# Chenxu1103/UNET-

Measured on AMD Instinct MI355X. Metric: frames/sec 512x512 3-class UNet++ inference; mask vs CPU reference, higher is better.
Workload: dtype f16 (MFMA operands split hi+lo, 3 MFMAs per product, f32 accumulate); 1 GPU; UNet++ 3-class 512x512 batch=16/GPU fp16-MFMA on 1 MI355X, synthetic frames, f32 NCHW in HBM -> uint8 mask in HBM; arch=nested, precision=exact, frames_per_gpu=16, global_batch=16, micro_batch=16, parallelism=frame-sharded x1, weights replicated (RCCL bcast)

## Files before the change

unet-_amd/csrc/tapmm_ws.h:

```cpp
#pragma once
#include "conv3x3_ws.h"

namespace unetpp {

struct TapmmArgs {
  const half_t* low;
  const half_t* wpk;
  float* y;
  int N, hw, K, Nv;
#ifdef UNETPP_WS_DBG
  int dbg;
#endif
};

struct TapmmCfg {
  static constexpr int NT = 512, NCONS = 4, NPROD = 4;
  static constexpr int TM = 256, TN = 128, MT = 4, NTL = 2;
  static constexpr int A_BYTES = TM * 64, B_BYTES = TN * 64, STAGE_BYTES = A_BYTES + B_BYTES;
  static constexpr int SLOTS = 6, LDS_BYTES = SLOTS * STAGE_BYTES;
  static constexpr int A_PIECES = A_BYTES / 1024, B_PIECES = B_BYTES / 1024;
  static constexpr int A_IT = A_PIECES / NPROD, B_IT = B_PIECES / NPROD, DMA_PER_STAGE = A_IT + B_IT;
  static constexpr int AHEAD = 4;
  static_assert(LDS_BYTES <= 160 * 1024 && AHEAD + 2 <= SLOTS, "ring");
};

template <bool X8>
__global__ __launch_bounds__(512, 2) void tapmm_ws_kernel(TapmmArgs a) {
  using C = TapmmCfg;
  extern __shared__ __attribute__((aligned(16))) char smem[];
  touch_kernarg_lines<TapmmArgs>();
  const int tid = threadIdx.x, lane = tid & 63;
  const int wave = __builtin_amdgcn_readfirstlane(tid >> 6);
  const unsigned lds_base = (unsigned)(unsigned long)(lds_char_t*)smem;
  const int mtiles_img = (a.hw + C::TM - 1) / C::TM;
  const int ntiles = a.Nv / C::TN;
  const int total_tiles = a.N * mtiles_img * ntiles;
  const int nst = a.K / 16;
  const int G = (int)gridDim.x;
  const int slot = (G % 8 == 0) ? ((int)blockIdx.x % 8) * (G / 8) + (int)blockIdx.x / 8 : (int)blockIdx.x;
  auto decode = [&](int t, int& n, int& q0, int& vt) {
    vt = t % ntiles; t /= ntiles;
    const int mt = t % mtiles_img;
    n = t / mtiles_img;
    q0 = mt * C::TM;
  };
  if (slot >= total_tiles) return;
  if (wave >= C::NCONS) {
    const int pw = wave - C::NCONS;
    constexpr unsigned OOB = 0x80000000u;
    const unsigned blk_bytes = (unsigned)a.hw * 64u;
    int it_tile = slot, it_s = 0;
    int in_, iq0, ivt;
    decode(it_tile, in_, iq0, ivt);
    auto issue = [&](int ring) {
#ifdef UNETPP_WS_DBG
      if (a.dbg & TAPMM_NO_DMA) {
        if (++it_s == nst) { it_s = 0; it_tile += G; if (it_tile < total_tiles) decode(it_tile, in_, iq0, ivt); }
        return;
      }
#endif
      const __amdgpu_buffer_rsrc_t rs = __builtin_amdgcn_make_buffer_rsrc(
          (void*)(a.low + (size_t)in_ * (a.K / 16) * a.hw * 32), 0, (int)((a.K / 16) * blk_bytes), 0x00020000);
      const unsigned dstA = lds_base + ring * C::STAGE_BYTES;
#pragma unroll
      for (int it = 0; it < C::A_IT; ++it) {
        const int piece = pw + it * C::NPROD;
        const int q = iq0 + piece * 16 + (lane & 15);
        const unsigned voff = q < a.hw ? (unsigned)q * 64u + (unsigned)(lane >> 4) * 16u : OOB;
        blds16(rs, voff, it_s * (int)blk_bytes, dstA + piece * 1024);
      }
      const char* wsrc = (const char*)a.wpk + ((size_t)ivt * nst + it_s) * C::B_BYTES;
#pragma unroll
      for (int it = 0; it < C::B_IT; ++it) {
        const int piece = pw + it * C::NPROD;
        glds16(wsrc + piece * 1024, lane * 16, dstA + C::A_BYTES + piece * 1024);
      }
      if (++it_s == nst) {
        it_s = 0; it_tile += G;
        if (it_tile < total_tiles) decode(it_tile, in_, iq0, ivt);
      }
    };
    int issued = 0, g = 0;
    for (int k = 0; k <= C::AHEAD && it_tile < total_tiles; ++k, ++issued) issue(issued % C::SLOTS);
    for (int tile = slot; tile < total_tiles; tile += G)
      for (int s = 0; s < nst; ++s, ++g) {
        const int later = issued - (g + 2);
        if (later >= 3) asm volatile("s_waitcnt vmcnt(18)" ::: "memory");
        else if (later == 2) asm volatile("s_waitcnt vmcnt(12)" ::: "memory");
        else if (later == 1) asm volatile("s_waitcnt vmcnt(6)" ::: "memory");
        else asm volatile("s_waitcnt vmcnt(0)" ::: "memory");
        lds_barrier();
        if (it_tile < total_tiles) { issue(issued % C::SLOTS); ++issued; }
      }
    return;
  }

  const int cw = wave, pxh = cw & 1, vh = cw >> 1;
  static_assert(C::DMA_PER_STAGE == 6, "vmcnt ladder above");
  int a_off[C::MT];
#pragma unroll
  for (int mt = 0; mt < C::MT; ++mt) {
    const int px = pxh * 128 + mt * 32 + (lane & 31);
    a_off[mt] = (px >> 4) * 1024 + ((lane >> 5) * 16 + (px & 15)) * 16;
  }
  const int b_off = C::A_BYTES + (vh * 2) * 2048 + (lane >> 5) * 512 + (lane & 31) * 16;
  struct Frag { half8 ah[C::MT], al[C::MT], bh[C::NTL], bl[C::NTL]; };
  auto load_frags = [&](Frag& f, int ring) {
    const char* st = smem + ring * C::STAGE_BYTES;
#pragma unroll
    for (int mt = 0; mt < C::MT; ++mt) { f.ah[mt] = *(const half8*)(st + a_off[mt]); f.al[mt] = *(const half8*)(st + a_off[mt] + 512); }
#pragma unroll
    for (int nt = 0; nt < C::NTL; ++nt) { f.bh[nt] = *(const half8*)(st + b_off + nt * 2048); f.bl[nt] = *(const half8*)(st + b_off + nt * 2048 + 1024); }
  };
  float16v acc[C::MT][C::NTL];
  auto run_mfma = [&](const Frag& f) {
    if (WS_OFF(a.dbg, TAPMM_NO_MFMA)) return;
#pragma unroll
    for (int mt = 0; mt < C::MT; ++mt)
#pragma unroll
      for (int nt = 0; nt < C::NTL; ++nt) {
        acc[mt][nt] = __builtin_amdgcn_mfma_f32_32x32x16_f16(f.bh[nt], f.al[mt], acc[mt][nt], 0, 0, 0);
        acc[mt][nt] = __builtin_amdgcn_mfma_f32_32x32x16_f16(f.bl[nt], f.ah[mt], acc[mt][nt], 0, 0, 0);
        acc[mt][nt] = __builtin_amdgcn_mfma_f32_32x32x16_f16(f.bh[nt], f.ah[mt], acc[mt][nt], 0, 0, 0);
      }
  };

  int g = 0;
  Frag f0, f1;
  bool have_f0 = false;
  struct HFrag { half8 a[C::MT], b[C::NTL]; };
  HFrag h0, h1;
  int8v xa[C::MT], xb[C::NTL];
  auto load_h = [&](HFrag& f, int ring) {
    const char* st = smem + ring * C::STAGE_BYTES;
#pragma unroll
    for (int mt = 0; mt < C::MT; ++mt) f.a[mt] = *(const half8*)(st + a_off[mt]);
#pragma unroll
    for (int nt = 0; nt < C::NTL; ++nt) f.b[nt] = *(const half8*)(st + b_off + nt * 2048);
  };
  auto load_x = [&](int ring0, int ring1) {
    const char* s0 = smem + ring0 * C::STAGE_BYTES;
    const char* s1 = smem + ring1 * C::STAGE_BYTES;
#pragma unroll
    for (int mt = 0; mt < C::MT; ++mt) {
      const int4v lo = *(const int4v*)(s0 + a_off[mt] + 512), hi = *(const int4v*)(s1 + a_off[mt] + 512);
      xa[mt] = __builtin_shufflevector(lo, hi, 0, 1, 2, 3, 4, 5, 6, 7);
    }
#pragma unroll
    for (int nt = 0; nt < C::NTL; ++nt) {
      const int4v lo = *(const int4v*)(s0 + b_off + nt * 2048 + 1024), hi = *(const int4v*)(s1 + b_off + nt * 2048 + 1024);
      xb[nt] = __builtin_shufflevector(lo, hi, 0, 1, 2, 3, 4, 5, 6, 7);
    }
  };
  auto main_mfma = [&](const HFrag& f) {
#pragma unroll
    for (int mt = 0; mt < C::MT; ++mt)
#pragma unroll
      for (int nt = 0; nt < C::NTL; ++nt) acc[mt][nt] = __builtin_amdgcn_mfma_f32_32x32x16_f16(f.b[nt], f.a[mt], acc[mt][nt], 0, 0, 0);
  };
  auto cross_mfma = [&]() {
#pragma unroll
    for (int mt = 0; mt < C::MT; ++mt)
#pragma unroll
      for (int nt = 0; nt < C::NTL; ++nt) {
        acc[mt][nt] = __builtin_amdgcn_mfma_scale_f32_32x32x64_f8f6f4(xb[nt], xa[mt], acc[mt][nt], 0 , 1 , 0, X8_SCALE_W, 0, X8_SCALE_A);
      }
  };
  for (int tile = slot; tile < total_tiles; tile += G) {
    int n, q0, vt;
    decode(tile, n, q0, vt);
#pragma unroll
    for (int mt = 0; mt < C::MT; ++mt)
#pragma unroll
      for (int nt = 0; nt < C::NTL; ++nt)
#pragma unroll
        for (int r = 0; r < 16; ++r) acc[mt][nt][r] = 0.f;
    const bool last_tile = tile + G >= total_tiles;
    if constexpr (X8) {
      for (int s = 0; s < nst; s += 2) {
        lds_barrier();
        if (!have_f0) { load_h(h0, g % C::SLOTS); have_f0 = true; }
        load_x(g % C::SLOTS, (g + 1) % C::SLOTS);
        load_h(h1, (g + 1) % C::SLOTS);
        __builtin_amdgcn_sched_barrier(0);
        main_mfma(h0);
        __builtin_amdgcn_sched_barrier(0);
        ++g;
        lds_barrier();
        const bool more = !(last_tile && s + 2 >= nst);
        if (more) load_h(h0, (g + 1) % C::SLOTS);
        have_f0 = more;
        __builtin_amdgcn_sched_barrier(0);
        cross_mfma();
        main_mfma(h1);
        __builtin_amdgcn_sched_barrier(0);
        ++g;
      }
    } else
    for (int s = 0; s < nst; s += 2) {
      lds_barrier();
      if (!have_f0) { load_frags(f0, g % C::SLOTS); have_f0 = true; }
      load_frags(f1, (g + 1) % C::SLOTS);
      __builtin_amdgcn_sched_barrier(0);
      run_mfma(f0);
      __builtin_amdgcn_sched_barrier(0);
      ++g;
      lds_barrier();
      const bool more = !(last_tile && s + 2 >= nst);
      if (more) load_frags(f0, (g + 1) % C::SLOTS);
      have_f0 = more;
      __builtin_amdgcn_sched_barrier(0);
      run_mfma(f1);
      __builtin_amdgcn_sched_barrier(0);
      ++g;
    }
    if (WS_OFF(a.dbg, TAPMM_NO_STORE)) { if (acc[0][0][0] == 12345.f) a.y[0] = 1.f; continue; }
    const int h = lane >> 5;
#pragma unroll
    for (int mt = 0; mt < C::MT; ++mt) {
      const int q = q0 + pxh * 128 + mt * 32 + (lane & 31);
#pragma unroll
      for (int nt = 0; nt < C::NTL; ++nt) {
        const int vb = vt * (C::TN / 32) + vh * 2 + nt;
        float* dst = a.y + (((size_t)n * (a.Nv / 32) + vb) * a.hw + q) * 32 + 4 * h;
        if (q < a.hw) {
#pragma unroll
          for (int qq = 0; qq < 4; ++qq) {
            *(f32x4*)(dst + 8 * qq) = (f32x4){acc[mt][nt][4 * qq], acc[mt][nt][4 * qq + 1], acc[mt][nt][4 * qq + 2], acc[mt][nt][4 * qq + 3]};
          }
        }
      }
    }
  }
}

__global__ void tapw_pack_kernel(const float* __restrict__ w, const float* __restrict__ mult, int Cout, int Cs, int Cup,
                                 half_t* __restrict__ out, long long units, int x8) {
  const long long u = (long long)blockIdx.x * blockDim.x + threadIdx.x;
  if (u >= units) return;
  long long t = u;
  const int vv = t % 32; t /= 32;
  const int kg = t % 2; t /= 2;
  const int pl = t % 2; t /= 2;
  const int vt = t % 4; t /= 4;
  const int nst = Cup / 16;
  const int ks = t % nst; t /= nst;
  const int v128 = (int)t;
  const int v = v128 * 128 + vt * 32 + vv;
  const int tap = v / Cout, co = v - tap * Cout;
  half8 r;
  float val[8];
#pragma unroll
  for (int e = 0; e < 8; ++e) {
    const int c = ks * 16 + kg * 8 + e;
    val[e] = w[((size_t)co * (Cs + Cup) + Cs + c) * 9 + tap] * mult[co];
    const half_t hi = (half_t)val[e];
    r[e] = pl == 0 ? hi : (half_t)(val[e] - (float)hi);
  }
  if (x8 && pl == 1) {
    unsigned wd[4];
#pragma unroll
    for (int q = 0; q < 2; ++q) {
      int a8 = 0, b8 = 0;
      float hi4[4], lo4[4];
#pragma unroll
      for (int i = 0; i < 4; ++i) { hi4[i] = val[4 * q + i] * 0.015625f; lo4[i] = (val[4 * q + i] - (float)(half_t)val[4 * q + i]) * 32.0f; }
      a8 = __builtin_amdgcn_cvt_pk_fp8_f32(hi4[0], hi4[1], a8, false); a8 = __builtin_amdgcn_cvt_pk_fp8_f32(hi4[2], hi4[3], a8, true);
      b8 = __builtin_amdgcn_cvt_pk_fp8_f32(lo4[0], lo4[1], b8, false); b8 = __builtin_amdgcn_cvt_pk_fp8_f32(lo4[2], lo4[3], b8, true);
      wd[2 * q] = (unsigned)a8; wd[2 * q + 1] = (unsigned)b8;
    }
    *(u32x4*)(out + u * 8) = (u32x4){wd[0], wd[1], wd[2], wd[3]};
    return;
  }
  *(half8*)(out + u * 8) = r;
}

struct UpsumArgs {
  const float* y;
  float* z;
  int N, H, W, Cout;
};

template <int TH_>
struct UpsumCfgT {
  static constexpr int TH = TH_, TW = 32, RH = TH / 2 + 3, RW = TW / 2 + 3, RECS = RH * RW;
  static constexpr int PIECES = (RECS * 128 + 1023) / 1024, BUF_BYTES = PIECES * 1024;
  static constexpr int YTAB_BYTES = (TH + 2) * 16, LDS_BYTES = BUF_BYTES + YTAB_BYTES;
  static constexpr int ITERS = (PIECES + 3) / 4;
};
typedef UpsumCfgT<16> UpsumCfg;

template <int TB, int TH_ = 16>
__global__ __launch_bounds__(256, TB == 1 ? 4 : 1) void upsum_kernel(UpsumArgs a) {
  using C = UpsumCfgT<TH_>;
  extern __shared__ __attribute__((aligned(16))) char smem[];
  const int H = a.H, W = a.W, h = H >> 1, w = W >> 1;
  const int tid = threadIdx.x, lane = tid & 63;
  const int wave = __builtin_amdgcn_readfirstlane(tid >> 6);
  const unsigned lds_base = (unsigned)(unsigned long)(lds_char_t*)smem;
  const int tiles_x = (W + C::TW - 1) / C::TW, tiles_y = (H + C::TH - 1) / C::TH;
  int t = blockIdx.x;
  const int tx = t % tiles_x; t /= tiles_x;
  const int ty = t % tiles_y; t /= tiles_y;
  const int cb = t % (a.Cout / 32);
  const int n = t / (a.Cout / 32);
  const int y0 = ty * C::TH, x0 = tx * C::TW;
  const float sh = h > 1 ? (float)(h - 1) / (float)(H - 1) : 0.f;
  const float sw = w > 1 ? (float)(w - 1) / (float)(W - 1) : 0.f;
  const int ybase = (int)(sh * (float)max(y0 - 1, 0)), xbase = (int)(sw * (float)max(x0 - 1, 0));
  const int vblocks = 9 * a.Cout / 32;
  const size_t plane = (size_t)h * w * 128;
  unsigned voff[C::ITERS];
#pragma unroll
  for (int it = 0; it < C::ITERS; ++it) {
    const int rec = (wave + it * 4) * 8 + (lane >> 3);
    const int ry = rec / C::RW, rx = rec - ry * C::RW;
    const int yy = min(ybase + ry, h - 1), xx = min(xbase + rx, w - 1);
    voff[it] = (wave + it * 4 < C::PIECES) ? (unsigned)((yy * w + xx) * 128 + (lane & 7) * 16) : 0x80000000u;
  }
  auto stage = [&](int tap, int buf) {
    const int vb = (tap * a.Cout) / 32 + cb;
    const __amdgpu_buffer_rsrc_t rs = __builtin_amdgcn_make_buffer_rsrc((void*)((const char*)a.y + ((size_t)n * vblocks + vb) * plane), 0,
                                                                       (int)plane, 0x00020000);
#pragma unroll
    for (int it = 0; it < C::ITERS; ++it) {
      const int piece = wave + it * 4;
      if (piece < C::PIECES) blds16(rs, voff[it], 0, lds_base + buf * C::BUF_BYTES + piece * 1024);
    }
  };
  const int cq = tid & 7, col = tid >> 3;
  int xo0[3], xo1[3]; float xl0[3], xl1[3];
#pragma unroll
  for (int dx = 0; dx < 3; ++dx) {
    const int xx = x0 + col + dx - 1;
    const bool in = xx >= 0 && xx < W && x0 + col < W;
    const float fx = sw * (float)max(xx, 0);
    const int c0 = min((int)fx, w - 1), c1 = c0 + (c0 < w - 1 ? 1 : 0);
    const float l1 = fminf(fmaxf(fx - (float)c0, 0.f), 1.f);
    xo0[dx] = min(max(c0 - xbase, 0), C::RW - 1) * 128 + cq * 16;
    xo1[dx] = min(max(c1 - xbase, 0), C::RW - 1) * 128 + cq * 16;
    xl0[dx] = in ? 1.f - l1 : 0.f; xl1[dx] = in ? l1 : 0.f;
  }
  struct YRow { int o0, o1; float l0, l1; };
  YRow* ytab = (YRow*)(smem + TB * C::BUF_BYTES);
  if (tid < C::TH + 2) {
    const int yy = y0 + tid - 1;
    const bool in = yy >= 0 && yy < H;
    const float fy = sh * (float)max(yy, 0);
    const int r0 = min((int)fy, h - 1), r1 = r0 + (r0 < h - 1 ? 1 : 0);
    const float l1 = fminf(fmaxf(fy - (float)r0, 0.f), 1.f);
    YRow e;
    e.o0 = min(max(r0 - ybase, 0), C::RH - 1) * (C::RW * 128);
    e.o1 = min(max(r1 - ybase, 0), C::RH - 1) * (C::RW * 128);
    e.l0 = in ? 1.f - l1 : 0.f; e.l1 = in ? l1 : 0.f;
    ytab[tid] = e;
  }
  f32x4 sum[C::TH];
#pragma unroll
  for (int r = 0; r < C::TH; ++r) sum[r] = (f32x4){0.f, 0.f, 0.f, 0.f};

  for (int tap0 = 0; tap0 < 9; tap0 += TB) {
    __syncthreads();
#pragma unroll
    for (int t = 0; t < TB; ++t) stage(tap0 + t, t);
    asm volatile("s_waitcnt vmcnt(0)" ::: "memory");
    __syncthreads();
#pragma unroll
    for (int t = 0; t < TB; ++t) {
    const int tap = tap0 + t;
    const char* reg = smem + t * C::BUF_BYTES;
    const int dy = tap / 3, dx = tap - dy * 3;
#pragma unroll
    for (int r = 0; r < C::TH; ++r) {
      const YRow yr = ytab[r + dy];
      const f32x4 c00 = *(const f32x4*)(reg + yr.o0 + xo0[dx]), c01 = *(const f32x4*)(reg + yr.o0 + xo1[dx]);
      const f32x4 c10 = *(const f32x4*)(reg + yr.o1 + xo0[dx]), c11 = *(const f32x4*)(reg + yr.o1 + xo1[dx]);
#pragma unroll
      for (int e = 0; e < 4; ++e) {
        const float t0 = fmaf(xl1[dx], c01[e], xl0[dx] * c00[e]), t1 = fmaf(xl1[dx], c11[e], xl0[dx] * c10[e]);
        sum[r][e] += fmaf(yr.l1, t1, yr.l0 * t0);
      }
    }
    }
  }
  const int x = x0 + col;
  if (x < W) {
#pragma unroll
    for (int r = 0; r < C::TH; ++r)
      if (y0 + r < H)
        *(f32x4*)(a.z + (((size_t)n * (a.Cout / 32) + cb) * ((size_t)H * W) + (size_t)(y0 + r) * W + x) * 32 + cq * 4) = sum[r];
  }
}

}
```

unet-_amd/csrc/unetpp_abi.hip:

```cpp
#include <hip/hip_runtime.h>

#include <algorithm>
#include <cerrno>
#include <cmath>
#include <cstdarg>
#include <cstdio>
#include <cstdlib>
#include <cstring>
#include <string>
#include <map>
#include <memory>
#include <mutex>
#include <set>
#include <tuple>
#include <utility>
#include <vector>

#include "abi_common.h"
#include "aux_kernels.h"
#include "conv3x3_mfma.h"
#include "conv3x3_ws.h"
#include "convt2x2_mfma.h"
#include "tapmm_ws.h"
#include "ws_dbg_host.h"
// ... 559 lines not shown
    snprintf(nm, sizeof nm, "dec%d", l + 1);
    int da = b.tensor(std::string(nm) + "a", SB[l], l);
    int d = b.tensor(nm, SB[l], l);
    int c1 = b.conv(std::string(nm) + ".0", 2 * SB[l], u, enc[l], da);
    e->convs[c1].w_off = dec_w[l][0]; e->convs[c1].b_off = dec_b[l][0];
    int c2 = b.conv(std::string(nm) + ".2", SB[l], da, -1, d);
    e->convs[c2].w_off = dec_w[l][1]; e->convs[c2].b_off = dec_b[l][1];
    prev = d;
  }
  b.off = off;
  b.head(prev, SB[0]);
}

struct Prec {
  int P; bool x8;
  template <class K> K pick(K fast, K exact, K exact8) const { return x8 ? exact8 : P == 2 ? exact : fast; }
  const char* args() const { return pick("1", "2", "2, true"); }
  const char* head_args() const { return pick("1", "2", "3"); }
};

struct InSlice { const char* raw; int format; double bytes_per_px; };
InSlice in_slice(const void* dev_input, int in_format, int b0, size_t hw) {
  const int bpp = in_format == UNETPP_IN_F32_NCHW ? 12 : 3;
  return {(const char*)dev_input + (size_t)b0 * hw * bpp, in_format, (double)bpp};
}

struct OutSlice {
  const unetpp_outputs* o = nullptr;
  float* logits = nullptr; float* probs = nullptr;
  uint8_t* mask = nullptr; uint8_t* cable = nullptr; uint8_t* tape = nullptr;
  double bytes_per_px = 0;
};
OutSlice out_slice(const unetpp_outputs* o, int b0, int C, size_t hw) {
  OutSlice r;
  if (!o) return r;
  r.o = o;
  if (o->dev_logits) r.logits = o->dev_logits + (size_t)b0 * C * hw;
  if (o->dev_probs) r.probs = o->dev_probs + (size_t)b0 * C * hw;
  if (o->dev_mask) r.mask = o->dev_mask + (size_t)b0 * hw;
  if (o->dev_cable) r.cable = o->dev_cable + (size_t)b0 * hw;
  if (o->dev_tape) r.tape = o->dev_tape + (size_t)b0 * hw;
  r.bytes_per_px = (r.logits ? 4.0 * C : 0) + (r.probs ? 4.0 * C : 0) + (r.mask ? 1 : 0) + (r.cable ? 1 : 0) + (r.tape ? 1 : 0);
  return r;
}

struct Pass {
  unetpp_engine* e;
  hipStream_t s;
  Launcher& lx;
  int nb, b0, h, w;
  int slot;
  size_t slot_off;
  InSlice in;
  OutSlice out[4];
  bool head_done = false;
#ifdef UNETPP_WS_DBG
  WsDbgPass dbg;
#endif
  half_t* tp(int id) const { return (half_t*)(e->arena + slot_off + e->tensors[id].off); }
};

bool x8_pair9(const unetpp_engine* e, const ConvLayer& L) { return e->x8 && L.nchunks % 2 == 0; }

void run_convert(Pass& c) {
  unetpp_engine* e = c.e;
  const Prec prec{e->P, e->x8};
  const size_t total = (size_t)c.nb * c.h * c.w;
  const double bytes = (double)total * c.in.bytes_per_px + (double)total * e->P * 16;
  c.lx.run(std::string("convert_input|convert_input_kernel<") + prec.args() + ">", 0, bytes, [&] {
    hipLaunchKernelGGL(prec.pick(convert_input_kernel<1>, convert_input_kernel<2>, convert_input_kernel<2, true>), dim3((unsigned)((total + 255) / 256)),
                       dim3(256), 0, c.s, (const void*)c.in.raw, c.in.format, c.nb, c.h, c.w, c.tp(e->t_in8), e->d_status);
    return hipSuccess;
  });
}

void run_conv(Pass& c, const Op& op) {
  unetpp_engine* e = c.e;
  const ConvLayer& L = e->convs[op.idx];
  const int P = e->P, C = e->cfg.num_classes;
  const bool head = op.fuse_head && !e->keep_all && L.cout == 32;
  const OutSlice& o = c.out[0];
  ConvArgs a{};
  const int H = c.h >> L.lvl, W = c.w >> L.lvl;
  const Tensor& t0 = e->tensors[L.in];
  const int c1 = L.in2 >= 0 ? e->tensors[L.in2].C : 0;
  a.in0 = c.tp(L.in); a.in1 = L.in2 >= 0 ? c.tp(L.in2) : nullptr; a.C0 = t0.C; a.C1 = c1;
  a.wpk = e->at<half_t>(L.wpk_at); a.scale = e->at<float>(L.scale_at); a.bias = e->blob + L.b_off; a.out = c.tp(L.out);
  a.pool_out = L.do_pool ? c.tp(L.pool) : nullptr;
  a.N = c.nb; a.H = H; a.W = W; a.Cout = L.cout;
  a.status = e->d_status;
  a.zinit = L.zt >= 0 ? (const float*)c.tp(L.zt) : nullptr;
  if (e->t_kpart >= 0) { a.kpart = (float*)c.tp(e->t_kpart); a.kcnt = (unsigned*)c.tp(e->t_kcnt); }
  a.ksplit = 1;
  a.pair9 = x8_pair9(e, L) ? 1 : 0;
  if (L.c0f) {
    const ConvLayer& L1 = e->convs[e->c0f_conv1];
    a.raw_in = c.in.raw;
    a.raw_fmt = c.in.format == UNETPP_IN_F32_NCHW ? 0 : 1;
    a.c1w = e->c1w; a.c1_scale = e->at<float>(L1.scale_at); a.c1_bias = e->blob + L1.b_off;
  }
  const int mw = small_grid_rows(L, e->num_cus, c.nb, H, W, head);
  const int TH = L.WAVES * mw;
  a.tiles_x = (W + 31) / 32; a.tiles_y = (H + TH - 1) / TH;
  a.nct = L.cout / (32 * L.NW); a.nchunks = L.nchunks;
  double px = (double)c.nb * H * W;
  double flops = 2.0 * px * L.cout * (L.zt >= 0 ? t0.C : L.cin_real) * 9;
  double bytes = px * P * 2.0 * (t0.C + (L.upf ? c1 / 4.0 : c1) + (head ? 0 : L.cout)) + (L.do_pool ? px / 4 * P * 2.0 * L.cout : 0.0) + (double)L.cout * L.cin_real * 9 * 2.0 * P;
  if (L.zt >= 0) bytes += px * L.cout * 4.0 - (double)L.cout * (L.cin_real - t0.C) * 9 * 2.0 * P;
  if (L.c0f) {
    flops += 2.0 * px * 32 * 3 * 9;
    bytes += px * c.in.bytes_per_px - px * P * 2.0 * t0.C;
  }
  if (head) {
    a.head_w = e->blob + e->head_w_off; a.head_b = e->blob + e->head_b_off; a.head_C = C;
    a.logits = o.logits; a.mask = o.mask; a.cable = o.cable; a.tape = o.tape;
    a.probs = o.probs; a.rule = o.o->rule;
    a.t_cable = o.o->t_cable; a.t_tape = o.o->t_tape; a.bg_margin = o.o->bg_margin; a.ct_margin = o.o->ct_margin;
    flops += 2.0 * px * 32 * C;
    bytes += px * o.bytes_per_px;
    c.head_done = true;
  }
  const WsVariant v = ws_variant(P, e->x8, L, head, e->keep_all);
  std::string lbl;
  if (L.ws) {
    lbl = ws_label(P, e->x8, L, v);
  } else {
    char buf[160];
    auto tf = [](bool b) { return b ? "true" : "false"; };
    snprintf(buf, sizeof buf, "%s%s%s|conv3x3_bias_relu_kernel<%d, %d, %d, %d, %d, %s, %s, %s>", L.name.c_str(), L.upf ? "+up" : "", head ? "+final+argmax" : "",
             P, L.KC, L.NW, mw, L.WAVES, tf(L.do_pool), tf(head), tf(L.upf));
    lbl = buf;
  }
#ifdef UNETPP_WS_DBG
  ws_dbg_before_launch(c.dbg, a, L.name, c.s);
#endif
  c.lx.run(lbl, flops, bytes, [&] {
    return L.ws ? launch_ws(LaunchCtx{e->cfg.device, e->num_cus, e->ksplit_max, e->ksplit_min_chunks, e->ksplit_gate, c.lx.plan}, e->x8, v, a, c.s)
                : launch_conv(LaunchCtx{e->cfg.device, e->num_cus, 1, 4, 4, c.lx.plan}, P, L, mw, a, head, c.s);
  });
#ifdef UNETPP_WS_DBG
  ws_dbg_after_launch(c.dbg, a, L.name, L.ws, c.s);
#endif
}

void run_tapmm(Pass& c, const Op& op) {
  unetpp_engine* e = c.e;
  const ConvLayer& L = e->convs[op.idx];
  const int P = e->P, H = c.h >> L.lvl, W = c.w >> L.lvl;
  const int cup = L.cin_real - e->tensors[L.in].C;
  TapmmArgs t{};
  t.low = c.tp(L.low_t); t.wpk = e->at<half_t>(L.tapw_at); t.y = (float*)c.tp(L.y_t);
  t.N = c.nb; t.hw = (H >> 1) * (W >> 1); t.K = cup; t.Nv = 9 * L.cout;
#ifdef UNETPP_WS_DBG
  { const char* d = getenv("UNETPP_TAPMM_DBG"); t.dbg = d ? atoi(d) : 0; }
#endif
  const int tiles = c.nb * ((t.hw + TapmmCfg::TM - 1) / TapmmCfg::TM) * (t.Nv / TapmmCfg::TN);
  const double M = (double)c.nb * t.hw;
  char lbl[96];
  snprintf(lbl, sizeof lbl, "%s.up-gemm|tapmm_ws_kernel<%s>", L.name.c_str(), e->x8 ? "true" : "false");
  c.lx.run(lbl, 2.0 * M * cup * t.Nv, M * cup * 2.0 * P + M * t.Nv * 4.0 + (double)t.Nv * cup * 2.0 * P, [&] {
    auto k = e->x8 ? tapmm_ws_kernel<true> : tapmm_ws_kernel<false>;
    hipError_t st = allow_full_lds((const void*)k, e->cfg.device);
    if (st != hipSuccess) return st;
    const int grid = std::min(tiles, e->num_cus);
    if (c.lx.plan) { c.lx.plan[0] = grid; c.lx.plan[1] = tiles; c.lx.plan[2] = 1; c.lx.plan[3] = 0; }
    hipLaunchKernelGGL(k, dim3((unsigned)grid), dim3(TapmmCfg::NT), TapmmCfg::LDS_BYTES, c.s, t);
    return hipSuccess;
  });
}

void run_upsum(Pass& c, const Op& op) {
  unetpp_engine* e = c.e;
  const ConvLayer& L = e->convs[op.idx];
  const int H = c.h >> L.lvl, W = c.w >> L.lvl;
  UpsumArgs u{};
  u.y = (const float*)c.tp(L.y_t); u.z = (float*)c.tp(L.zt); u.N = c.nb; u.H = H; u.W = W; u.Cout = L.cout;
  unsigned blocks = (unsigned)(((W + UpsumCfg::TW - 1) / UpsumCfg::TW) * ((H + UpsumCfg::TH - 1) / UpsumCfg::TH) * (L.cout / 32) * c.nb);
  const double px = (double)c.nb * H * W;
  char lbl[96];
  const bool small = blocks <= (unsigned)e->num_cus;
  if (small) blocks = (unsigned)(((W + 31) / 32) * ((H + 3) / 4) * (L.cout / 32) * c.nb);
  snprintf(lbl, sizeof lbl, "%s.up-sum|upsum_kernel<1, %d>", L.name.c_str(), small ? 4 : 16);
  c.lx.run(lbl, px * L.cout * 9 * 8.0, px / 4 * 9 * L.cout * 4.0 + px * L.cout * 4.0, [&] {
    if (small) hipLaunchKernelGGL((upsum_kernel<1, 4>), dim3(blocks), dim3(256), UpsumCfgT<4>::LDS_BYTES, c.s, u);
    else hipLaunchKernelGGL((upsum_kernel<1, 16>), dim3(blocks), dim3(256), UpsumCfg::LDS_BYTES, c.s, u);
    return hipSuccess;
  });
}

void run_up(Pass& c, const Op& op) {
  unetpp_engine* e = c.e;
  const Tensor& low = e->tensors[op.idx];
  const Tensor& dst = e->tensors[op.out];
  const int P = e->P, H = c.h >> dst.lvl, W = c.w >> dst.lvl;
  double px = (double)c.nb * H * W;
  double bytes = px * P * 2.0 * low.C + px / 4 * P * 2.0 * low.C;
  const int nseg = (W + UP_SEG - 1) / UP_SEG;
  const int seg_w = std::min(W, UP_SEG);
  const size_t up_lds = (size_t)3 * (seg_w / 2 + 2) * P * 32;
  const int up_threads = seg_w * 2 * P >= 1024 ? 512 : (seg_w * 2 * P >= 256 ? 256 : 128);
  char nm[64];
  snprintf(nm, sizeof nm, "up%d|upsample2x_kernel<1>", dst.lvl);
  c.lx.run(nm, px * low.C * 8, bytes, [&] {
    if (P != 1) return hipErrorInvalidValue;
    hipLaunchKernelGGL(upsample2x_kernel<1>, dim3((unsigned)((H / 2) * nseg), (unsigned)(c.nb * (low.C / 16))), dim3(up_threads), up_lds, c.s, c.tp(op.idx), H, W, c.tp(op.out));
    return hipSuccess;
  });
}

void run_convt(Pass& c, const Op& op) {
  unetpp_engine* e = c.e;
  const ConvTLayer& T = e->convts[op.idx];
  const Prec prec{e->P, e->x8};
  const int P = e->P, H = c.h >> T.lvl, W = c.w >> T.lvl;
  ConvTArgs a{};
  a.in = c.tp(T.in); a.wpk = e->at<half_t>(T.wpk_at); a.scale = e->at<float>(T.scale_at); a.bias = e->blob + T.b_off; a.out = c.tp(T.out);
  a.N = c.nb; a.H = H; a.W = W; a.Cin = T.cin; a.Cout = T.cout;
  a.status = e->d_status;
  double px = (double)c.nb * H * W;
  double flops = 2.0 * px * T.cin * T.cout * 4;
  double bytes = px * P * 2.0 * (T.cin + 4.0 * T.cout) + 4.0 * T.cin * T.cout * 2.0 * P;
  dim3 grid((unsigned)(((H * W + 511) / 512) * (4 * T.cout / 64) * c.nb));
  c.lx.run(T.name + "|convt2x2_kernel<" + prec.args() + ">", flops, bytes, [&] {
    hipLaunchKernelGGL(prec.pick(convt2x2_kernel<1>, convt2x2_kernel<2>, convt2x2_kernel<2, true>), grid, dim3(256), 0, c.s, a);
    return hipSuccess;
  });
}

void run_ds(Pass& c, const Op& op) {
  unetpp_engine* e = c.e;
  const Prec prec{e->P, e->x8};
  const int k = op.idx, C = e->cfg.num_classes, P = e->P, h = c.h, w = c.w;
  const OutSlice& o = c.out[k];
  if (!o.o) return;
  const int cx = e->tensors[op.out].C, hk = h >> k, wk = w >> k;
  const double lowpx = (double)c.nb * hk * wk, px = (double)c.nb * h * w;
  const float* dsw = e->ds_w + e->ds_w_off[k];
  const char* nm = k == 3 ? "ds3_1" : k == 2 ? "ds2_2" : "ds1_3";
  float* low = e->ds_scratch[c.slot] + e->ds_scr_off[k];
  const dim3 hgrid((unsigned)((hk * wk + 255) / 256), (unsigned)c.nb);
  const size_t lds = (size_t)(C * cx + C) * sizeof(float);
  c.lx.run(std::string(nm) + "|head_generic_kernel<" + prec.head_args() + ">", 2.0 * lowpx * cx * C, lowpx * (P * 2.0 * cx + 4.0 * C), [&] {
    uint8_t* none = nullptr;
    hipLaunchKernelGGL(prec.pick(head_generic_kernel<1>, head_generic_kernel<2>, head_generic_kernel<3>), hgrid, dim3(256), lds, c.s, c.tp(op.out), cx, dsw,
                       dsw + (size_t)C * cx, C, hk, wk, low, (float*)nullptr, none, none, none, 0, 0.f, 0.f, 0.f, 0.f);
    return hipSuccess;
  });
  const float sy = (float)(hk - 1) / (float)(h - 1), sx = (float)(wk - 1) / (float)(w - 1);
  const size_t items = (size_t)c.nb * h * (w / 4);
  c.lx.run(std::string(nm) + "+up|ds_upsample_kernel", px * C * 9.0, lowpx * 4.0 * C + px * o.bytes_per_px, [&] {
    hipLaunchKernelGGL(ds_upsample_kernel, dim3((unsigned)((items + 255) / 256)), dim3(256), 0, c.s, (const float*)low, C, hk, wk, c.nb, h, w, sy, sx,
                       o.logits, o.probs, o.mask, o.cable, o.tape, o.o->rule, o.o->t_cable, o.o->t_tape, o.o->bg_margin, o.o->ct_margin);
    return hipSuccess;
  });
}

void run_head(Pass& c, const Op& op) {
  if (c.head_done) return;
  unetpp_engine* e = c.e;
  const Prec prec{e->P, e->x8};
  const OutSlice& o = c.out[0];
  const int cx = e->head_cx, C = e->cfg.num_classes;
  const size_t hw = (size_t)c.h * c.w, total = c.nb * hw;
  const dim3 grid((unsigned)((hw + 255) / 256), (unsigned)c.nb);
  const size_t lds = (size_t)(C * cx + C) * sizeof(float);
  c.lx.run(std::string("final+argmax|head_generic_kernel<") + prec.head_args() + ">", 2.0 * total * cx * C, (double)total * (e->P * 2.0 * cx + o.bytes_per_px), [&] {
    hipLaunchKernelGGL(prec.pick(head_generic_kernel<1>, head_generic_kernel<2>, head_generic_kernel<3>), grid, dim3(256), lds, c.s, c.tp(op.out), cx,
                       e->blob + e->head_w_off, e->blob + e->head_b_off, C, c.h, c.w, o.logits, o.probs, o.mask, o.cable, o.tape, o.o->rule, o.o->t_cable,
                       o.o->t_tape, o.o->bg_margin, o.o->ct_margin);
    return hipSuccess;
  });
}

}

extern "C" {

#ifndef UNETPP_SRC_HASH
#define UNETPP_SRC_HASH "unknown"
#endif
#ifdef UNETPP_WS_DBG
#define UNETPP_BUILD_TAG " +wsdbg"
#else
#define UNETPP_BUILD_TAG ""
#endif
const char* unetpp_version(void) { return "unetpp-hip 0.3.0 (gfx950) src:" UNETPP_SRC_HASH UNETPP_BUILD_TAG; }

const char* unetpp_last_error(const unetpp_engine* e) { return e ? e->err.c_str() : g_create_error.c_str(); }

size_t unetpp_weights_blob_bytes(int num_classes, int in_channels) {
  return 32 + 4 * blob_payload_floats(UNETPP_ARCH_NESTED, num_classes, in_channels);
}

size_t unetpp_weights_blob_bytes_arch(int arch, int num_classes, int in_channels) {
  if (arch != UNETPP_ARCH_NESTED && arch != UNETPP_ARCH_SIMPLE) return 0;
  return 32 + 4 * blob_payload_floats(arch, num_classes, in_channels);
}

int unetpp_create(const unetpp_config* cfg, unetpp_engine** out) {
  if (!cfg || !out) return fail(nullptr, UNETPP_E_INVALID, "null argument");
  *out = nullptr;
  if (cfg->arch != UNETPP_ARCH_NESTED && cfg->arch != UNETPP_ARCH_SIMPLE) return fail(nullptr, UNETPP_E_INVALID, "arch=%d unknown", cfg->arch);
  if (cfg->in_channels != 3) return fail(nullptr, UNETPP_E_UNSUPPORTED, "input_channels=%d unsupported (only 3)", cfg->in_channels);
  if (cfg->num_classes < 1 || cfg->num_classes > HEAD_FUSED_MAX_CLASSES)
    return fail(nullptr, UNETPP_E_INVALID, "num_classes=%d out of range [1,%d]", cfg->num_classes, HEAD_FUSED_MAX_CLASSES);
  const int mult = cfg->arch == UNETPP_ARCH_NESTED ? 16 : 8;
  if (cfg->max_batch < 1 || cfg->max_h < mult || cfg->max_w < mult || cfg->max_h % mult || cfg->max_w % mult)
// ... 445 lines not shown
```

Before: 4276 frames/s.

## Block tapmm tiles for L2 weight reuse and overlap epilogue stores with MFMAs

When the grid size is a multiple of 8, tapmm tiles are remapped so that each XCD-group of blocks walks a limited band of weight column tiles sized to about 2.5MB, aiming to keep weights resident in L2. Accumulator zeroing is folded into the first MFMA by passing a zero accumulator. Output stores become bounds-checked buffer stores interleaved with the last k-step's MFMAs, so the write-out overlaps compute. A second kernel's tile order is also remapped to group tiles per XCD with y as the fast axis. The changes add index arithmetic and scheduling complexity, and the store interleave depends on sched_barrier placement.

```diff
diff --git a/unet-_amd/csrc/tapmm_ws.h b/unet-_amd/csrc/tapmm_ws.h
--- a/unet-_amd/csrc/tapmm_ws.h
+++ b/unet-_amd/csrc/tapmm_ws.h
@@ -22,6 +22,7 @@
   static constexpr int A_IT = A_PIECES / NPROD, B_IT = B_PIECES / NPROD, DMA_PER_STAGE = A_IT + B_IT;
   static constexpr int AHEAD = 4;
   static_assert(LDS_BYTES <= 160 * 1024 && AHEAD + 2 <= SLOTS, "ring");
+  static constexpr long long W_L2 = 5 << 19;
 };
 
 template <bool X8>
@@ -38,8 +39,19 @@
   const int nst = a.K / 16;
   const int G = (int)gridDim.x;
   const int slot = (G % 8 == 0) ? ((int)blockIdx.x % 8) * (G / 8) + (int)blockIdx.x / 8 : (int)blockIdx.x;
+  const int nblk = (int)(((long long)ntiles * a.K * (C::TN * 4) + C::W_L2 - 1) / C::W_L2);
+  const int vblk = (ntiles + nblk - 1) / nblk;
+  const bool blocked = G % 8 == 0 && vblk < ntiles;
   auto decode = [&](int t, int& n, int& q0, int& vt) {
-    vt = t % ntiles; t /= ntiles;
+    if (blocked) {
+      const int g8 = G / 8, s = t % G, x = s / g8, rounds = total_tiles / G, rem = total_tiles - rounds * G;
+      const int p = x * rounds * g8 + min(rem, x * g8) + (t / G) * g8 + (s - x * g8);
+      const int span = vblk * a.N * mtiles_img, vb = p / span, r = p - vb * span;
+      const int wd = min(vblk, ntiles - vb * vblk);
+      vt = vb * vblk + r % wd; t = r / wd;
+    } else {
+      vt = t % ntiles; t /= ntiles;
+    }
     const int mt = t % mtiles_img;
     n = t / mtiles_img;
     q0 = mt * C::TM;
@@ -113,16 +125,33 @@
     for (int nt = 0; nt < C::NTL; ++nt) { f.bh[nt] = *(const half8*)(st + b_off + nt * 2048); f.bl[nt] = *(const half8*)(st + b_off + nt * 2048 + 1024); }
   };
   float16v acc[C::MT][C::NTL];
-  auto run_mfma = [&](const Frag& f) {
-    if (WS_OFF(a.dbg, TAPMM_NO_MFMA)) return;
-#pragma unroll
-    for (int mt = 0; mt < C::MT; ++mt)
-#pragma unroll
-      for (int nt = 0; nt < C::NTL; ++nt) {
-        acc[mt][nt] = __builtin_amdgcn_mfma_f32_32x32x16_f16(f.bh[nt], f.al[mt], acc[mt][nt], 0, 0, 0);
-        acc[mt][nt] = __builtin_amdgcn_mfma_f32_32x32x16_f16(f.bl[nt], f.ah[mt], acc[mt][nt], 0, 0, 0);
-        acc[mt][nt] = __builtin_amdgcn_mfma_f32_32x32x16_f16(f.bh[nt], f.ah[mt], acc[mt][nt], 0, 0, 0);
-      }
+  const float16v zero16 = {0.f, 0.f, 0.f, 0.f, 0.f, 0.f, 0.f, 0.f, 0.f, 0.f, 0.f, 0.f, 0.f, 0.f, 0.f, 0.f};
+  const float* yplane = a.y;
+  int yvoff = 0;
+  auto store_part = [&](int i, int qq) {
+    if (WS_OFF(a.dbg, TAPMM_NO_STORE)) return;
+    const int mt = i / C::NTL, nt = i % C::NTL;
+    const __amdgpu_buffer_rsrc_t rs = __builtin_amdgcn_make_buffer_rsrc((void*)(yplane + (size_t)nt * a.hw * 32), 0, a.hw * 128, 0x00020000);
+    __builtin_amdgcn_raw_buffer_store_b128(
+        __builtin_bit_cast(u32x4, (f32x4){acc[mt][nt][4 * qq], acc[mt][nt][4 * qq + 1], acc[mt][nt][4 * qq + 2], acc[mt][nt][4 * qq + 3]}),
+        rs, yvoff + mt * (32 * 128) + qq * 32, 0, 0);
+  };
+  auto run_mfma = [&](const Frag& f, auto first, bool fin) {
+    constexpr bool FIRST = decltype(first)::value;
+    const bool mm = !WS_OFF(a.dbg, TAPMM_NO_MFMA);
+#pragma unroll
+    for (int i = 0; i < C::MT * C::NTL; ++i) {
+      const int mt = i / C::NTL, nt = i % C::NTL;
+      if (FIRST && !mm) acc[mt][nt] = zero16;
+      if (mm) acc[mt][nt] = __builtin_amdgcn_mfma_f32_32x32x16_f16(f.bh[nt], f.al[mt], FIRST ? zero16 : acc[mt][nt], 0, 0, 0);
+      if (mm) acc[mt][nt] = __builtin_amdgcn_mfma_f32_32x32x16_f16(f.bl[nt], f.ah[mt], acc[mt][nt], 0, 0, 0);
+      if (fin && i > 0) { store_part(i - 1, 0); store_part(i - 1, 1); }
+      if (mm) acc[mt][nt] = __builtin_amdgcn_mfma_f32_32x32x16_f16(f.bh[nt], f.ah[mt], acc[mt][nt], 0, 0, 0);
+      if (fin && i > 0) { store_part(i - 1, 2); store_part(i - 1, 3); }
+    }
+    if (fin)
+#pragma unroll
+      for (int qq = 0; qq < 4; ++qq) store_part(C::MT * C::NTL - 1, qq);
   };
 
   int g = 0;
@@ -152,11 +181,19 @@
       xb[nt] = __builtin_shufflevector(lo, hi, 0, 1, 2, 3, 4, 5, 6, 7);
     }
   };
-  auto main_mfma = [&](const HFrag& f) {
-#pragma unroll
-    for (int mt = 0; mt < C::MT; ++mt)
-#pragma unroll
-      for (int nt = 0; nt < C::NTL; ++nt) acc[mt][nt] = __builtin_amdgcn_mfma_f32_32x32x16_f16(f.b[nt], f.a[mt], acc[mt][nt], 0, 0, 0);
+  auto main_mfma = [&](const HFrag& f, auto first, bool fin) {
+    constexpr bool FIRST = decltype(first)::value;
+#pragma unroll
+    for (int i = 0; i < C::MT * C::NTL; ++i) {
+      const int mt = i / C::NTL, nt = i % C::NTL;
+      acc[mt][nt] = __builtin_amdgcn_mfma_f32_32x32x16_f16(f.b[nt], f.a[mt], FIRST ? zero16 : acc[mt][nt], 0, 0, 0);
+      if (fin && i > 0)
+#pragma unroll
+        for (int qq = 0; qq < 4; ++qq) store_part(i - 1, qq);
+    }
+    if (fin)
+#pragma unroll
+      for (int qq = 0; qq < 4; ++qq) store_part(C::MT * C::NTL - 1, qq);
   };
   auto cross_mfma = [&]() {
 #pragma unroll
@@ -169,12 +206,8 @@
   for (int tile = slot; tile < total_tiles; tile += G) {
     int n, q0, vt;
     decode(tile, n, q0, vt);
-#pragma unroll
-    for (int mt = 0; mt < C::MT; ++mt)
-#pragma unroll
-      for (int nt = 0; nt < C::NTL; ++nt)
-#pragma unroll
-        for (int r = 0; r < 16; ++r) acc[mt][nt][r] = 0.f;
+    yplane = a.y + ((size_t)n * (a.Nv / 32) + vt * (C::TN / 32) + vh * 2) * a.hw * 32;
+    yvoff = (q0 + pxh * 128 + (lane & 31)) * 128 + (lane >> 5) * 16;
     const bool last_tile = tile + G >= total_tiles;
     if constexpr (X8) {
       for (int s = 0; s < nst; s += 2) {
@@ -183,16 +216,17 @@
         load_x(g % C::SLOTS, (g + 1) % C::SLOTS);
         load_h(h1, (g + 1) % C::SLOTS);
         __builtin_amdgcn_sched_barrier(0);
-        main_mfma(h0);
+        if (s == 0) main_mfma(h0, std::true_type{}, false); else main_mfma(h0, std::false_type{}, false);
         __builtin_amdgcn_sched_barrier(0);
         ++g;
         lds_barrier();
-        const bool more = !(last_tile && s + 2 >= nst);
+        const bool fin = s + 2 >= nst;
+        const bool more = !(last_tile && fin);
         if (more) load_h(h0, (g + 1) % C::SLOTS);
         have_f0 = more;
         __builtin_amdgcn_sched_barrier(0);
         cross_mfma();
-        main_mfma(h1);
+        main_mfma(h1, std::false_type{}, fin);
         __builtin_amdgcn_sched_barrier(0);
         ++g;
       }
@@ -202,35 +236,20 @@
       if (!have_f0) { load_frags(f0, g % C::SLOTS); have_f0 = true; }
       load_frags(f1, (g + 1) % C::SLOTS);
       __builtin_amdgcn_sched_barrier(0);
-      run_mfma(f0);
+      if (s == 0) run_mfma(f0, std::true_type{}, false); else run_mfma(f0, std::false_type{}, false);
       __builtin_amdgcn_sched_barrier(0);
       ++g;
       lds_barrier();
-      const bool more = !(last_tile && s + 2 >= nst);
+      const bool fin = s + 2 >= nst;
+      const bool more = !(last_tile && fin);
       if (more) load_frags(f0, (g + 1) % C::SLOTS);
       have_f0 = more;
       __builtin_amdgcn_sched_barrier(0);
-      run_mfma(f1);
+      run_mfma(f1, std::false_type{}, fin);
       __builtin_amdgcn_sched_barrier(0);
       ++g;
     }
-    if (WS_OFF(a.dbg, TAPMM_NO_STORE)) { if (acc[0][0][0] == 12345.f) a.y[0] = 1.f; continue; }
-    const int h = lane >> 5;
-#pragma unroll
-    for (int mt = 0; mt < C::MT; ++mt) {
-      const int q = q0 + pxh * 128 + mt * 32 + (lane & 31);
-#pragma unroll
-      for (int nt = 0; nt < C::NTL; ++nt) {
-        const int vb = vt * (C::TN / 32) + vh * 2 + nt;
-        float* dst = a.y + (((size_t)n * (a.Nv / 32) + vb) * a.hw + q) * 32 + 4 * h;
-        if (q < a.hw) {
-#pragma unroll
-          for (int qq = 0; qq < 4; ++qq) {
-            *(f32x4*)(dst + 8 * qq) = (f32x4){acc[mt][nt][4 * qq], acc[mt][nt][4 * qq + 1], acc[mt][nt][4 * qq + 2], acc[mt][nt][4 * qq + 3]};
-          }
-        }
-      }
-    }
+    if (WS_OFF(a.dbg, TAPMM_NO_STORE) && acc[0][0][0] == 12345.f) a.y[0] = 1.f;
   }
 }
 
@@ -299,9 +318,13 @@
   const int wave = __builtin_amdgcn_readfirstlane(tid >> 6);
   const unsigned lds_base = (unsigned)(unsigned long)(lds_char_t*)smem;
   const int tiles_x = (W + C::TW - 1) / C::TW, tiles_y = (H + C::TH - 1) / C::TH;
-  int t = blockIdx.x;
-  const int tx = t % tiles_x; t /= tiles_x;
-  const int ty = t % tiles_y; t /= tiles_y;
+  const int G = (int)gridDim.x;
+  const bool runs = G % 8 == 0;
+  int t = runs ? ((int)blockIdx.x % 8) * (G / 8) + (int)blockIdx.x / 8 : (int)blockIdx.x;
+  const int fast = runs ? tiles_y : tiles_x, slow = runs ? tiles_x : tiles_y;
+  const int tf = t % fast; t /= fast;
+  const int ts = t % slow; t /= slow;
+  const int tx = runs ? ts : tf, ty = runs ? tf : ts;
   const int cb = t % (a.Cout / 32);
   const int n = t / (a.Cout / 32);
   const int y0 = ty * C::TH, x0 = tx * C::TW;
diff --git a/unet-_amd/csrc/unetpp_abi.hip b/unet-_amd/csrc/unetpp_abi.hip
--- a/unet-_amd/csrc/unetpp_abi.hip
+++ b/unet-_amd/csrc/unetpp_abi.hip
@@ -735,7 +735,8 @@
   t.low = c.tp(L.low_t); t.wpk = e->at<half_t>(L.tapw_at); t.y = (float*)c.tp(L.y_t);
   t.N = c.nb; t.hw = (H >> 1) * (W >> 1); t.K = cup; t.Nv = 9 * L.cout;
 #ifdef UNETPP_WS_DBG
-  { const char* d = getenv("UNETPP_TAPMM_DBG"); t.dbg = d ? atoi(d) : 0; }
+  { const char* d = getenv("UNETPP_TAPMM_DBG"); t.dbg = d ? atoi(d) : 0;
+    const char* only = getenv("UNETPP_TAPMM_DBG_LAYER"); if (only && !strstr(L.name.c_str(), only)) t.dbg = 0; }
 #endif
   const int tiles = c.nb * ((t.hw + TapmmCfg::TM - 1) / TapmmCfg::TM) * (t.Nv / TapmmCfg::TN);
   const double M = (double)c.nb * t.hw;
```

Measured after the change: 4303 frames/s (median of 6 runs). About the same (+0.6%).
